# nianticlabs/wavelet-monodepth

Hardware: AMD Instinct MI355X
Metric: decoder+IDWT frames/sec @640x192 bs12 (higher is better)
Workload: dtype f32; 1 GPU; KITTI ResNet18 640x192 dense wavelet decoder + 4x Haar IDWT, forward, batch 12 per GPU (BASELINE.json configs[1]); encoder features resident in HBM; batch_per_gpu=12, global_batch=12, parallelism=dp1 (independent shards)

## Files before the change

### include/wmd.h

```cpp
#ifndef WMD_H
#define WMD_H

#include <stddef.h>
#include <stdint.h>

#ifdef __cplusplus
extern "C" {
#endif

#define WMD_VERSION 100

typedef enum {
    WMD_OK = 0,
    WMD_ERR_BAD_ARG = -1,
    WMD_ERR_BAD_SHAPE = -2,
    WMD_ERR_UNSUPPORTED = -3,
    WMD_ERR_HIP = -4,
    WMD_ERR_WORKSPACE = -5,
    WMD_ERR_COMM = -6
} wmd_status;

typedef enum { WMD_PAD_ZERO = 0, WMD_PAD_REFLECT = 1, WMD_PAD_REPLICATE = 2 } wmd_pad;

typedef enum { WMD_ACT_NONE = 0, WMD_ACT_ELU = 1, WMD_ACT_LEAKY = 2, WMD_ACT_SIGMOID = 3 } wmd_act;
// ... 27 lines not shown
    int B, H, W;
    int C1;
    int up1;
    int C2;
    int Cout;
    int ksize;
    int pad_mode;
    int act;
    float slope;
    const float* x1;
    const float* x2;
    const float* wp;
    const float* bias;
    float* y;
    float* workspace;
    size_t workspace_floats;
    int tune_cfg;
    int tune_ksplit;
    const float* wp_wino;
    const float* gate;
    int gate_act;
    float gate_slope;
    const uint8_t* in_mask;
    const uint8_t* out_mask;
    int in_mask_2x2;
    const int32_t* out_tiles;
    const int32_t* out_tile_count;
    int out_tile_h, out_tile_w;
} wmd_conv_args;

int wmd_conv_list_tile_supported(int tile_h, int tile_w);

int wmd_conv_fwd(const wmd_conv_args* args, void* stream);

size_t wmd_conv_fwd_workspace_floats(const wmd_conv_args* args);

size_t wmd_conv_packed_weight_floats_wino(int Cout, int Cin);
int wmd_conv_pack_weights_wino(const float* w, float* wp, int Cout, int Cin, int dgrad, void* stream);

typedef struct {
    const float* w;
    int Cout, Cin, ksize;
    float* fwd;
    float* dgrad;
    float* wino_fwd;
    float* wino_dgrad;
} wmd_pack_item;
int wmd_conv_pack_many(const wmd_pack_item* items, int n, void* stream);

int wmd_conv_num_configs(void);
const char* wmd_conv_config_name(int i);

size_t wmd_conv_bf16_packed_weight_bytes(int Cout, int Cin, int terms);
int wmd_conv_bf16_pack_weights(const float* w, void* wp, int Cout, int Cin, int terms, void* stream);
int wmd_conv_bf16_supported(const wmd_conv_args* args, int terms);
size_t wmd_conv_bf16_workspace_floats(const wmd_conv_args* args, int terms);
int wmd_conv_bf16_fwd(const wmd_conv_args* args, int terms, void* stream);
int wmd_conv_bf16_num_configs(void);
const char* wmd_conv_bf16_config_name(int i);

int wmd_act_bwd(const float* dy, const float* y, float* dz, size_t n, int act, float slope, void* stream);

typedef struct {
    int B, H, W;
    int C1, up1, C2, Cout, ksize, pad_mode;
    const float* dz;
    const float* wp_dgrad;
    float* dx1;
    float* dx2;
    float* workspace;
    size_t workspace_floats;
    int tune_cfg;
    int tune_ksplit;
    const float* wp_dgrad_wino;
    const float* x1_fwd;
    int x1_act;
    float x1_slope;
} wmd_conv_dgrad_args;

size_t wmd_conv_dgrad_workspace_floats(const wmd_conv_dgrad_args* args);
int wmd_conv_dgrad(const wmd_conv_dgrad_args* args, void* stream);

typedef struct {
    int B, H, W;
    int C1, up1, C2, Cout, ksize, pad_mode;
    const float* x1;
    const float* x2;
    const float* dz;
    float* dw;
    float* dbias;
    float* workspace;
    size_t workspace_floats;
    int tune_cfg;
    int tune_nsplit;
} wmd_conv_wgrad_args;

int wmd_conv_wgrad_num_configs(void);
const char* wmd_conv_wgrad_config_name(int index);

size_t wmd_conv_wgrad_workspace_floats(const wmd_conv_wgrad_args* args);
int wmd_conv_wgrad(const wmd_conv_wgrad_args* args, void* stream);

typedef struct {
    int B, H, W;
    int C1, up1, C2, pad_mode;
    const float* x1;
    const float* x2;
    const float* w;
} wmd_dwconv_args;
int wmd_dwconv3x3_fwd(const wmd_dwconv_args* args, float* y, void* stream);
size_t wmd_dwconv3x3_bwd_workspace_floats(const wmd_dwconv_args* args);
int wmd_dwconv3x3_bwd(const wmd_dwconv_args* args, const float* y, const float* dy, float* dx1, float* dx2, float* dw,
                      float* workspace, size_t workspace_floats, void* stream);

typedef struct {
    int B, H, W, C;
    int Cout;
    int pad_mode;
    int mode;
    float scale;
    const float* xp; const float* wgt_p; const float* bias_p;
    const float* xn; const float* wgt_n; const float* bias_n;
    float* y;
    float* sig_p;
    float* sig_n;
    size_t xp_bstride;
    size_t xn_bstride;
    float* workspace;
    size_t workspace_floats;
} wmd_head_args;

int wmd_head3x3_fwd(const wmd_head_args* args, void* stream);
size_t wmd_head3x3_workspace_floats(const wmd_head_args* args);

typedef struct {
    int B, H, W, C;
    float slope;
    const float* x;
    const float* wp1;
    const float* bias1;
    const float* wp2;
    float* t;
    int chain;
    int t_planes;
    const uint8_t* run_mask;
    const float* ll_wp1;
    const float* ll_bias1;
    const float* ll_wp2;
    float* mid_out;
    int mid_ct, mid_off_p, mid_off_n, mid_off_ll;
} wmd_head_fused_args;
int wmd_head_fused_fwd(const wmd_head_fused_args* args, void* stream);
int wmd_head_fused_multi_fwd(const wmd_head_fused_args* levels, int n_levels, void* stream);

typedef struct {
    int B, H, W;
    int pad_mode;
    float scale;
    const float* t;
    const float* bias_p;
    const float* bias_n;
    float* yh;
    const float* yl;
    float* out;
    float* disp;
    float disp_scale;
    int clamp01;
    const float* bias_ll;
    float scale_ll;
    float* yl_out;
    const uint8_t* yh_mask;
    uint32_t* range_keys;
    float* sig_p;
    float* sig_n;
    float* sig_ll;
} wmd_head_shiftsum_args;
int wmd_head_shiftsum_fwd(const wmd_head_shiftsum_args* args, void* stream);
int wmd_head_shiftsum_chain_fwd(const wmd_head_shiftsum_args* levels, int n_levels, void* stream);

typedef struct {
    int B, H, W, C;
    int pad_mode;
    float slope;
    float scale;
    const float* x;
    const float* wp1;
    const float* bias1;
    const float* wp2;
    const float* bias_p;
    const float* bias_n;
    float* yh;
    const float* yl;
    float* out;
    float* disp;
    float disp_scale;
    int clamp01;
    const uint8_t* yh_mask;
    float* mid_out;
    int mid_ct, mid_off_p, mid_off_n;
    float* sig_p;
    float* sig_n;
} wmd_head_level_args;
int wmd_head_level_supported(int C);
int wmd_head_level_fwd(const wmd_head_level_args* args, void* stream);
int wmd_head_level_pyramid_supported(int C, int B, int H, int W);
int wmd_head_level_pyramid_fwd(const wmd_head_level_args* args, const wmd_head_shiftsum_args* coarse, int n_coarse, void* stream);

typedef struct {
    int row0;
    int nrows;
    int ch0;
    int nch;
    const float* w3;
    float* dw3;
    float* db3;
} wmd_head_bwd_head;
typedef struct {
    int B, H, W;
    int Ct;
    int n_out;
    int pad_mode;
    int act;
    float slope;
    const float* dy3;
    const float* mid;
    float* dzmid;
    int n_heads;
    wmd_head_bwd_head head[3];
    float* workspace;
    size_t workspace_floats;
} wmd_head3x3_bwd_args;
size_t wmd_head3x3_bwd_workspace_floats(const wmd_head3x3_bwd_args* args);
int wmd_head3x3_bwd(const wmd_head3x3_bwd_args* args, void* stream);

typedef struct {
    int B, H, W;
    int C;
    int Ct;
    int x_act;
    float x_slope;
    const float* dz;
    const float* x;
    const float* w1;
    float* dx;
    float* dw1;
    float* db1;
    float* workspace;
    size_t workspace_floats;
} wmd_head1x1_bwd_args;
size_t wmd_head1x1_bwd_workspace_floats(const wmd_head1x1_bwd_args* args);
int wmd_head1x1_bwd(const wmd_head1x1_bwd_args* args, void* stream);
int wmd_head_bwd(const wmd_head3x3_bwd_args* a3, const wmd_head1x1_bwd_args* a1, void* stream);


int wmd_minmax(const float* x, size_t n, float* out2, void* stream);

int wmd_mask_threshold(const float* yh, const float* minmax, float thresh_ratio, uint8_t* mask,
                       int h, int w, void* stream);

typedef struct {
    int up;
    int radius;
    uint8_t* out;
    int32_t* nnz;
    int nnz_stride;
} wmd_dilate_spec;
int wmd_mask_dilate_multi(const uint8_t* mask, int h, int w, const wmd_dilate_spec* specs, int n, void* stream);
int wmd_mask_dilate_multi_b(const uint8_t* mask, int B, int h, int w, const wmd_dilate_spec* specs, int n, void* stream);

int wmd_mask_level(const float* yl, size_t n_yl, const float* yh, float thresh_ratio, int h, int w,
                   const wmd_dilate_spec* specs, int n, void* stream);
int wmd_mask_level_b(const float* yl, size_t n_yl, const float* yh, float thresh_ratio, int B, int h, int w,
                     const wmd_dilate_spec* specs, int n, float* minmax_scratch, void* stream);

typedef struct {
    int up, radius;
    uint8_t* out;
    int count;
    int tile_h, tile_w;
    int32_t* tile_list;
    int32_t* tile_count;
    const uint8_t* and_mask;
} wmd_level_spec;

typedef struct {
    int B, h, w;
    const float* yl;
    size_t n_yl;
    const float* yh;
    float thresh_ratio;
    const uint8_t* mask0;
    const float* minmax;
    uint32_t* range_keys;
    const wmd_level_spec* specs;
    int n;
    int32_t* scratch;
    int32_t* counts;
    int ring_slots, slot_ints, counts_off, ncounts;
    int advance;
} wmd_mask_level_args;
size_t wmd_mask_level_scratch_ints(int B);
int wmd_mask_level_lists(const wmd_mask_level_args* args, void* stream);

typedef struct {
    const uint8_t* mask;
    int npix;
// ... 99 lines not shown
```

### wavelet_monodepth_amd/_lib.py

```python
import ctypes as C
import os

_HERE = os.path.dirname(os.path.abspath(__file__))
LIB_PATH = os.environ.get("WMD_LIB_PATH") or os.path.join(_HERE, "libwmd_hip.so")

PAD = {"zero": 0, "constant": 0, "reflect": 1, "reflection": 1, "replicate": 2}
ACT = {"none": 0, None: 0, "elu": 1, "leaky": 2, "sigmoid": 3}


class WmdError(RuntimeError):
    pass


class ConvArgs(C.Structure):
    _fields_ = [("B", C.c_int), ("H", C.c_int), ("W", C.c_int), ("C1", C.c_int), ("up1", C.c_int), ("C2", C.c_int),
                ("Cout", C.c_int), ("ksize", C.c_int), ("pad_mode", C.c_int), ("act", C.c_int), ("slope", C.c_float),
                ("x1", C.c_void_p), ("x2", C.c_void_p), ("wp", C.c_void_p), ("bias", C.c_void_p), ("y", C.c_void_p),
                ("workspace", C.c_void_p), ("workspace_floats", C.c_size_t), ("tune_cfg", C.c_int), ("tune_ksplit", C.c_int),
                ("wp_wino", C.c_void_p), ("gate", C.c_void_p), ("gate_act", C.c_int), ("gate_slope", C.c_float),
                ("in_mask", C.c_void_p), ("out_mask", C.c_void_p), ("in_mask_2x2", C.c_int),
                ("out_tiles", C.c_void_p), ("out_tile_count", C.c_void_p), ("out_tile_h", C.c_int), ("out_tile_w", C.c_int)]


class ConvDgradArgs(C.Structure):
# ... 9 lines not shown
                ("Cout", C.c_int), ("ksize", C.c_int), ("pad_mode", C.c_int),
                ("x1", C.c_void_p), ("x2", C.c_void_p), ("dz", C.c_void_p), ("dw", C.c_void_p), ("dbias", C.c_void_p),
                ("workspace", C.c_void_p), ("workspace_floats", C.c_size_t), ("tune_cfg", C.c_int), ("tune_nsplit", C.c_int)]


class HeadArgs(C.Structure):
    _fields_ = [("B", C.c_int), ("H", C.c_int), ("W", C.c_int), ("C", C.c_int), ("Cout", C.c_int),
                ("pad_mode", C.c_int), ("mode", C.c_int), ("scale", C.c_float),
                ("xp", C.c_void_p), ("wgt_p", C.c_void_p), ("bias_p", C.c_void_p),
                ("xn", C.c_void_p), ("wgt_n", C.c_void_p), ("bias_n", C.c_void_p),
                ("y", C.c_void_p), ("sig_p", C.c_void_p), ("sig_n", C.c_void_p),
                ("xp_bstride", C.c_size_t), ("xn_bstride", C.c_size_t),
                ("workspace", C.c_void_p), ("workspace_floats", C.c_size_t)]


class HeadFusedArgs(C.Structure):
    _fields_ = [("B", C.c_int), ("H", C.c_int), ("W", C.c_int), ("C", C.c_int), ("slope", C.c_float),
                ("x", C.c_void_p), ("wp1", C.c_void_p), ("bias1", C.c_void_p), ("wp2", C.c_void_p), ("t", C.c_void_p),
                ("chain", C.c_int), ("t_planes", C.c_int), ("run_mask", C.c_void_p), ("ll_wp1", C.c_void_p),
                ("ll_bias1", C.c_void_p), ("ll_wp2", C.c_void_p), ("mid_out", C.c_void_p), ("mid_ct", C.c_int),
                ("mid_off_p", C.c_int), ("mid_off_n", C.c_int), ("mid_off_ll", C.c_int)]


class HeadLevelArgs(C.Structure):
    _fields_ = [("B", C.c_int), ("H", C.c_int), ("W", C.c_int), ("C", C.c_int), ("pad_mode", C.c_int),
                ("slope", C.c_float), ("scale", C.c_float),
                ("x", C.c_void_p), ("wp1", C.c_void_p), ("bias1", C.c_void_p), ("wp2", C.c_void_p),
                ("bias_p", C.c_void_p), ("bias_n", C.c_void_p), ("yh", C.c_void_p),
                ("yl", C.c_void_p), ("out", C.c_void_p), ("disp", C.c_void_p), ("disp_scale", C.c_float),
                ("clamp01", C.c_int), ("yh_mask", C.c_void_p), ("mid_out", C.c_void_p), ("mid_ct", C.c_int),
                ("mid_off_p", C.c_int), ("mid_off_n", C.c_int), ("sig_p", C.c_void_p), ("sig_n", C.c_void_p)]


class HeadBwdHead(C.Structure):
    _fields_ = [("row0", C.c_int), ("nrows", C.c_int), ("ch0", C.c_int), ("nch", C.c_int), ("w3", C.c_void_p),
                ("dw3", C.c_void_p), ("db3", C.c_void_p)]


class Head3x3BwdArgs(C.Structure):
    _fields_ = [("B", C.c_int), ("H", C.c_int), ("W", C.c_int), ("Ct", C.c_int), ("n_out", C.c_int), ("pad_mode", C.c_int),
                ("act", C.c_int), ("slope", C.c_float), ("dy3", C.c_void_p), ("mid", C.c_void_p), ("dzmid", C.c_void_p),
                ("n_heads", C.c_int), ("head", HeadBwdHead * 3), ("workspace", C.c_void_p), ("workspace_floats", C.c_size_t)]


class Head1x1BwdArgs(C.Structure):
    _fields_ = [("B", C.c_int), ("H", C.c_int), ("W", C.c_int), ("C", C.c_int), ("Ct", C.c_int), ("x_act", C.c_int),
                ("x_slope", C.c_float), ("dz", C.c_void_p), ("x", C.c_void_p), ("w1", C.c_void_p), ("dx", C.c_void_p),
                ("dw1", C.c_void_p), ("db1", C.c_void_p), ("workspace", C.c_void_p), ("workspace_floats", C.c_size_t)]


class EvalKittiArgs(C.Structure):
    _fields_ = [("B", C.c_int), ("h", C.c_int), ("w", C.c_int), ("H", C.c_int), ("W", C.c_int),
                ("min_depth", C.c_float), ("max_depth", C.c_float), ("mask_mode", C.c_int), ("pred_scale", C.c_float),
                ("median_scaling", C.c_int), ("pred_disp", C.c_void_p), ("gt_depth", C.c_void_p), ("out", C.c_void_p),
                ("workspace", C.c_void_p), ("workspace_floats", C.c_size_t)]


class WarpArgs(C.Structure):
    _fields_ = [("B", C.c_int), ("C", C.c_int), ("H", C.c_int), ("W", C.c_int), ("Hs", C.c_int), ("Ws", C.c_int),
                ("eps", C.c_float), ("src", C.c_void_p), ("depth", C.c_void_p), ("K", C.c_void_p), ("inv_K", C.c_void_p),
                ("T", C.c_void_p)]


class DwConvArgs(C.Structure):
    _fields_ = [("B", C.c_int), ("H", C.c_int), ("W", C.c_int), ("C1", C.c_int), ("up1", C.c_int), ("C2", C.c_int),
                ("pad_mode", C.c_int), ("x1", C.c_void_p), ("x2", C.c_void_p), ("w", C.c_void_p)]


class HeadShiftsumArgs(C.Structure):
    _fields_ = [("B", C.c_int), ("H", C.c_int), ("W", C.c_int), ("pad_mode", C.c_int), ("scale", C.c_float),
                ("t", C.c_void_p), ("bias_p", C.c_void_p), ("bias_n", C.c_void_p), ("yh", C.c_void_p),
                ("yl", C.c_void_p), ("out", C.c_void_p), ("disp", C.c_void_p), ("disp_scale", C.c_float),
                ("clamp01", C.c_int), ("bias_ll", C.c_void_p), ("scale_ll", C.c_float), ("yl_out", C.c_void_p),
                ("yh_mask", C.c_void_p), ("range_keys", C.c_void_p), ("sig_p", C.c_void_p), ("sig_n", C.c_void_p),
                ("sig_ll", C.c_void_p)]


class LevelSpec(C.Structure):
    _fields_ = [("up", C.c_int), ("radius", C.c_int), ("out", C.c_void_p), ("count", C.c_int), ("tile_h", C.c_int),
                ("tile_w", C.c_int), ("tile_list", C.c_void_p), ("tile_count", C.c_void_p), ("and_mask", C.c_void_p)]


class MaskLevelArgs(C.Structure):
    _fields_ = [("B", C.c_int), ("h", C.c_int), ("w", C.c_int), ("yl", C.c_void_p), ("n_yl", C.c_size_t), ("yh", C.c_void_p),
                ("thresh_ratio", C.c_float), ("mask0", C.c_void_p), ("minmax", C.c_void_p), ("range_keys", C.c_void_p),
                ("specs", C.POINTER(LevelSpec)), ("n", C.c_int), ("scratch", C.c_void_p), ("counts", C.c_void_p),
                ("ring_slots", C.c_int), ("slot_ints", C.c_int), ("counts_off", C.c_int), ("ncounts", C.c_int),
                ("advance", C.c_int)]


class DilateSpec(C.Structure):
    _fields_ = [("up", C.c_int), ("radius", C.c_int), ("out", C.c_void_p), ("nnz", C.c_void_p), ("nnz_stride", C.c_int)]


class PackItem(C.Structure):
    _fields_ = [("w", C.c_void_p), ("Cout", C.c_int), ("Cin", C.c_int), ("ksize", C.c_int), ("fwd", C.c_void_p),
                ("dgrad", C.c_void_p), ("wino_fwd", C.c_void_p), ("wino_dgrad", C.c_void_p)]


class CompactSpec(C.Structure):
    _fields_ = [("mask", C.c_void_p), ("npix", C.c_int), ("coords", C.c_void_p), ("nnz", C.c_void_p)]


class SparseConvArgs(C.Structure):
    _fields_ = [("H", C.c_int), ("W", C.c_int), ("C1", C.c_int), ("up1", C.c_int), ("C1tot", C.c_int), ("c1_off", C.c_int),
                ("C2", C.c_int), ("Cout", C.c_int), ("ksize", C.c_int), ("pad_mode", C.c_int), ("act", C.c_int),
                ("slope", C.c_float), ("x1", C.c_void_p), ("x2", C.c_void_p), ("in_mask", C.c_void_p),
                ("out_coords", C.c_void_p), ("out_nnz", C.c_void_p), ("max_out", C.c_int),
                ("wp", C.c_void_p), ("bias", C.c_void_p), ("wp2", C.c_void_p), ("bias2", C.c_void_p),
                ("c1_off2", C.c_int), ("out_scale", C.c_float), ("y", C.c_void_p), ("split_waves", C.c_int),
                ("B", C.c_int), ("nnz_stride", C.c_int)]


_lib = None

SIGNATURES = {
    "wmd_version": (C.c_int, []),
    "wmd_last_error": (C.c_char_p, []),
    "wmd_status_string": (C.c_char_p, [C.c_int]),
    "wmd_profile_begin": (C.c_int, []),
    "wmd_profile_end": (C.c_long, [C.c_char_p, C.c_size_t]),
    "wmd_idwt_haar_fwd": (C.c_int, [C.c_void_p] * 4 + [C.c_int] * 3 + [C.c_float, C.c_int, C.c_void_p]),
    "wmd_idwt_haar_bwd": (C.c_int, [C.c_void_p] * 5 + [C.c_int] * 3 + [C.c_float, C.c_int, C.c_void_p]),
    "wmd_dwt_haar_fwd": (C.c_int, [C.c_void_p] * 3 + [C.c_int] * 3 + [C.c_void_p]),
    "wmd_dwt_haar_reflect_fwd": (C.c_int, [C.c_void_p] * 3 + [C.c_int] * 3 + [C.c_void_p]),
    "wmd_conv_packed_weight_floats": (C.c_size_t, [C.c_int] * 3),
    "wmd_conv_pack_weights": (C.c_int, [C.c_void_p, C.c_void_p, C.c_int, C.c_int, C.c_int, C.c_void_p]),
    "wmd_conv_pack_weights_dgrad": (C.c_int, [C.c_void_p, C.c_void_p, C.c_int, C.c_int, C.c_int, C.c_void_p]),
    "wmd_conv_packed_weight_floats_wino": (C.c_size_t, [C.c_int, C.c_int]),
    "wmd_conv_pack_weights_wino": (C.c_int, [C.c_void_p, C.c_void_p, C.c_int, C.c_int, C.c_int, C.c_void_p]),
    "wmd_conv_pack_many": (C.c_int, [C.c_void_p, C.c_int, C.c_void_p]),
    "wmd_conv_fwd": (C.c_int, [C.POINTER(ConvArgs), C.c_void_p]),
    "wmd_conv_fwd_workspace_floats": (C.c_size_t, [C.POINTER(ConvArgs)]),
    "wmd_conv_num_configs": (C.c_int, []),
    "wmd_conv_config_name": (C.c_char_p, [C.c_int]),
    "wmd_conv_bf16_packed_weight_bytes": (C.c_size_t, [C.c_int] * 3),
    "wmd_conv_bf16_pack_weights": (C.c_int, [C.c_void_p, C.c_void_p, C.c_int, C.c_int, C.c_int, C.c_void_p]),
    "wmd_conv_bf16_supported": (C.c_int, [C.POINTER(ConvArgs), C.c_int]),
    "wmd_conv_bf16_workspace_floats": (C.c_size_t, [C.POINTER(ConvArgs), C.c_int]),
    "wmd_conv_bf16_fwd": (C.c_int, [C.POINTER(ConvArgs), C.c_int, C.c_void_p]),
    "wmd_conv_bf16_num_configs": (C.c_int, []),
    "wmd_conv_bf16_config_name": (C.c_char_p, [C.c_int]),
    "wmd_act_bwd": (C.c_int, [C.c_void_p] * 3 + [C.c_size_t, C.c_int, C.c_float, C.c_void_p]),
    "wmd_conv_dgrad_workspace_floats": (C.c_size_t, [C.POINTER(ConvDgradArgs)]),
    "wmd_conv_dgrad": (C.c_int, [C.POINTER(ConvDgradArgs), C.c_void_p]),
    "wmd_conv_wgrad_workspace_floats": (C.c_size_t, [C.POINTER(ConvWgradArgs)]),
    "wmd_conv_wgrad": (C.c_int, [C.POINTER(ConvWgradArgs), C.c_void_p]),
    "wmd_conv_wgrad_num_configs": (C.c_int, []),
    "wmd_conv_wgrad_config_name": (C.c_char_p, [C.c_int]),
    "wmd_head3x3_fwd": (C.c_int, [C.POINTER(HeadArgs), C.c_void_p]),
    "wmd_head3x3_workspace_floats": (C.c_size_t, [C.POINTER(HeadArgs)]),
    "wmd_head_fused_fwd": (C.c_int, [C.POINTER(HeadFusedArgs), C.c_void_p]),
    "wmd_head_fused_multi_fwd": (C.c_int, [C.POINTER(HeadFusedArgs), C.c_int, C.c_void_p]),
    "wmd_head_shiftsum_fwd": (C.c_int, [C.POINTER(HeadShiftsumArgs), C.c_void_p]),
    "wmd_head_shiftsum_chain_fwd": (C.c_int, [C.POINTER(HeadShiftsumArgs), C.c_int, C.c_void_p]),
    "wmd_head_level_supported": (C.c_int, [C.c_int]),
    "wmd_head_level_fwd": (C.c_int, [C.POINTER(HeadLevelArgs), C.c_void_p]),
    "wmd_head_level_pyramid_supported": (C.c_int, [C.c_int, C.c_int, C.c_int, C.c_int]),
    "wmd_head_level_pyramid_fwd": (C.c_int, [C.POINTER(HeadLevelArgs), C.POINTER(HeadShiftsumArgs), C.c_int, C.c_void_p]),
    "wmd_head3x3_bwd_workspace_floats": (C.c_size_t, [C.POINTER(Head3x3BwdArgs)]),
    "wmd_head3x3_bwd": (C.c_int, [C.POINTER(Head3x3BwdArgs), C.c_void_p]),
    "wmd_head1x1_bwd_workspace_floats": (C.c_size_t, [C.POINTER(Head1x1BwdArgs)]),
    "wmd_head1x1_bwd": (C.c_int, [C.POINTER(Head1x1BwdArgs), C.c_void_p]),
    "wmd_head_bwd": (C.c_int, [C.POINTER(Head3x3BwdArgs), C.POINTER(Head1x1BwdArgs), C.c_void_p]),
    "wmd_minmax": (C.c_int, [C.c_void_p, C.c_size_t, C.c_void_p, C.c_void_p]),
    "wmd_mask_threshold": (C.c_int, [C.c_void_p, C.c_void_p, C.c_float, C.c_void_p, C.c_int, C.c_int, C.c_void_p]),
    "wmd_mask_dilate_multi": (C.c_int, [C.c_void_p, C.c_int, C.c_int, C.POINTER(DilateSpec), C.c_int, C.c_void_p]),
    "wmd_mask_level": (C.c_int, [C.c_void_p, C.c_size_t, C.c_void_p, C.c_float, C.c_int, C.c_int, C.POINTER(DilateSpec), C.c_int,
                       C.c_void_p]),
    "wmd_mask_compact_multi": (C.c_int, [C.POINTER(CompactSpec), C.c_int, C.c_void_p]),
    "wmd_mask_dilate_multi_b": (C.c_int, [C.c_void_p, C.c_int, C.c_int, C.c_int, C.POINTER(DilateSpec), C.c_int, C.c_void_p]),
    "wmd_mask_level_b": (C.c_int, [C.c_void_p, C.c_size_t, C.c_void_p, C.c_float, C.c_int, C.c_int, C.c_int, C.POINTER(DilateSpec), C.c_int,
                         C.c_void_p, C.c_void_p]),
    "wmd_mask_compact_multi_b": (C.c_int, [C.POINTER(CompactSpec), C.c_int, C.c_int, C.c_void_p]),
    "wmd_mask_level_scratch_ints": (C.c_size_t, [C.c_int]),
    "wmd_mask_level_lists": (C.c_int, [C.POINTER(MaskLevelArgs), C.c_void_p]),
    "wmd_conv_list_tile_supported": (C.c_int, [C.c_int, C.c_int]),
    "wmd_sparse_conv": (C.c_int, [C.POINTER(SparseConvArgs), C.c_void_p]),
    "wmd_upsample_bilinear_fwd": (C.c_int, [C.c_void_p] * 3 + [C.c_int] * 6 + [C.c_float, C.c_float, C.c_void_p]),
    "wmd_upsample_bilinear_bwd": (C.c_int, [C.c_void_p] * 4 + [C.c_int] * 6 + [C.c_float, C.c_float, C.c_void_p]),
    "wmd_eval_workspace_floats": (C.c_size_t, [C.c_int, C.c_int, C.c_int]),
    "wmd_eval_kitti": (C.c_int, [C.POINTER(EvalKittiArgs), C.c_void_p]),
    "wmd_eval_errors": (C.c_int, [C.c_void_p, C.c_void_p, C.c_int, C.c_size_t, C.c_void_p, C.c_void_p]),
    "wmd_flip_postprocess": (C.c_int, [C.c_void_p, C.c_void_p, C.c_void_p, C.c_int, C.c_int, C.c_int, C.c_void_p]),
    "wmd_ssim_fwd": (C.c_int, [C.c_void_p] * 3 + [C.c_int] * 5 + [C.c_float, C.c_float, C.c_void_p]),
    "wmd_ssim_bwd_workspace_floats": (C.c_size_t, [C.c_int] * 4),
    "wmd_ssim_bwd": (C.c_int, [C.c_void_p] * 5 + [C.c_int] * 5 + [C.c_float, C.c_float, C.c_void_p, C.c_size_t, C.c_void_p]),
    "wmd_warp_fwd": (C.c_int, [C.POINTER(WarpArgs), C.c_void_p, C.c_void_p]),
    "wmd_warp_bwd_workspace_floats": (C.c_size_t, [C.POINTER(WarpArgs)]),
    "wmd_warp_bwd": (C.c_int, [C.POINTER(WarpArgs), C.c_void_p, C.c_void_p, C.c_void_p, C.c_void_p, C.c_size_t, C.c_void_p]),
    "wmd_smooth_workspace_floats": (C.c_size_t, [C.c_int] * 3),
    "wmd_smooth_fwd": (C.c_int, [C.c_void_p] * 3 + [C.c_int] * 4 + [C.c_float, C.c_void_p, C.c_size_t, C.c_void_p]),
    "wmd_smooth_bwd": (C.c_int, [C.c_void_p] * 4 + [C.c_int] * 4 + [C.c_float, C.c_void_p]),
    "wmd_dwconv3x3_fwd": (C.c_int, [C.POINTER(DwConvArgs), C.c_void_p, C.c_void_p]),
    "wmd_dwconv3x3_bwd_workspace_floats": (C.c_size_t, [C.POINTER(DwConvArgs)]),
    "wmd_dwconv3x3_bwd": (C.c_int, [C.POINTER(DwConvArgs)] + [C.c_void_p] * 6 + [C.c_size_t, C.c_void_p]),
    "wmd_comm_unique_id": (C.c_int, [C.c_void_p]),
    "wmd_comm_init": (C.c_int, [C.POINTER(C.c_void_p), C.c_void_p, C.c_int, C.c_int]),
    "wmd_comm_allreduce": (C.c_int, [C.c_void_p, C.c_void_p, C.c_size_t, C.c_float, C.c_void_p]),
    "wmd_comm_broadcast": (C.c_int, [C.c_void_p, C.c_void_p, C.c_size_t, C.c_int, C.c_void_p]),
    "wmd_comm_info": (C.c_int, [C.c_void_p, C.POINTER(C.c_int), C.POINTER(C.c_int), C.POINTER(C.c_int)]),
    "wmd_comm_destroy": (C.c_int, [C.c_void_p]),
}


def lib():
    global _lib
    if _lib is None:
        if not os.path.exists(LIB_PATH):
            raise WmdError("%s not found: build it with `python -m wavelet_monodepth_amd.build` "
                           "(or __graft_entry__.build()); there is no CPU fallback" % LIB_PATH)
        handle = C.CDLL(LIB_PATH)
        for name, (res, args) in SIGNATURES.items():
            fn = getattr(handle, name)
            fn.restype = res
            fn.argtypes = args
        _lib = handle
    return _lib


def check(status, what=""):
    if status != 0:
        l = lib()
        raise WmdError("%s failed: %s (%s)" % (what or "libwmd_hip call", l.wmd_status_string(status).decode(),
                                               l.wmd_last_error().decode()))


def ptr(t):
    if t is None:
        return None
    if not t.is_cuda:
        raise WmdError("libwmd_hip expects device tensors, got a %s tensor" % t.device)
    assert t.is_contiguous(), "libwmd_hip expects contiguous tensors"
    return t.data_ptr()


def current_stream():
    import torch

    return torch.cuda.current_stream().cuda_stream


def profile_begin():
    check(lib().wmd_profile_begin(), "wmd_profile_begin")


def profile_end():
    import json

    buf = C.create_string_buffer(1 << 16)
    n = lib().wmd_profile_end(buf, len(buf))
    if n < 0:
        check(int(n), "wmd_profile_end")
    return json.loads(buf.value.decode())
```

### wavelet_monodepth_amd/csrc/wmd_head_chain.hip

```cpp
#include <algorithm>
#include <cstdlib>
#include <type_traits>
#include <utility>
#include "wmd_internal.h"

#ifndef WMD_CHAIN_PD256
#define WMD_CHAIN_PD256 4
#endif
#ifndef WMD_CHAIN_PD128
#define WMD_CHAIN_PD128 1
#endif

namespace wmd {

typedef float f32x4 __attribute__((ext_vector_type(4)));

template <class F, int... I>
__device__ __forceinline__ void hc_static_for_impl(F&& f, std::integer_sequence<int, I...>) {
    (f(std::integral_constant<int, I>{}), ...);
}
template <int N, class F>
__device__ __forceinline__ void hc_static_for(F&& f) {
    hc_static_for_impl(f, std::make_integer_sequence<int, N>{});
}

__device__ __forceinline__ void hc_barrier() {
    asm volatile("s_waitcnt lgkmcnt(0)" ::: "memory");
    __builtin_amdgcn_s_barrier();
    asm volatile("" ::: "memory");
}

struct HeadChainArgs {
    const float* x;
    const float* wp1;
    const float* bias1;
    const float* wp2;
    float* t;
    int plane, tiles, t_planes;
    int C;
    float slope;
    const uint8_t* run_mask;
    const float* ll_wp1;
    const float* ll_bias1;
    const float* ll_wp2;
    float* mid_out;
    int mid_ct, mid_off[3];
};

template <int C, int RS, int PG, int NT, int KC>
struct HeadChainTile {
    static constexpr int NW = RS * PG, NTH = NW * 64;
    static constexpr int PXB = PG * NT * 16;
    static constexpr int MTS = C / 16;
    static constexpr int MT = MTS / RS;
    static constexpr int KS = C / 4;
    static constexpr int NCH = KS / KC;
    static constexpr int XS = PXB % 32 == 0 ? PXB + 16 : PXB + 32;
    static constexpr int WF = MTS * KC * 64;
    static constexpr int XF = KC * 4 * XS;
    static constexpr int NBUF = NCH > 1 ? 2 : 1;
    static constexpr int WV = (WF / 4 + NTH - 1) / NTH;
    static constexpr int XV = (KC * PXB + NTH - 1) / NTH;
    static constexpr int RED = RS > 1 ? NW * 3 * NT * 256 : 0;
    static constexpr int WFL = (C == 256 && RS == 4) ? RS * KC * 64 : 0;
    static constexpr int STAGE = NBUF * (WF + WFL + XF);
    static constexpr int LDS_FLOATS = STAGE > RED ? STAGE : RED;
    static_assert(C % 16 == 0 && MTS % RS == 0 && KS % KC == 0, "whole tiles");
    static_assert(XS % 32 == 16 && PXB % 4 == 0, "bank-conflict-free x rows");
};

template <class T, int KC, bool LLX>
__device__ __forceinline__ void chain_fetch(f32x4 (&wreg)[T::WV], f32x4 (&xreg)[T::XV], f32x4& lreg, const float* __restrict__ w1,
                                            const float* __restrict__ wl, const float* __restrict__ xb, int c, int tid, int pix0, int plane) {
    if constexpr (LLX) {
        static_assert(T::WFL > 0 && T::WFL / 4 <= T::NTH, "one 16-byte piece per thread covers the low-pass part of a chunk");
        const int f = tid * 4, m = f / (KC * 64), rem = f % (KC * 64);
        if (f < T::WFL) lreg = *reinterpret_cast<const f32x4*>(wl + ((size_t)m * T::KS + c * KC) * 64 + rem);
    }
#pragma unroll
    for (int v = 0; v < T::WV; ++v) {
        const int f = (v * T::NTH + tid) * 4;
        const int m = f / (KC * 64), rem = f % (KC * 64);
        f32x4 wv = {0.f, 0.f, 0.f, 0.f};
        if (T::WF % (4 * T::NTH) == 0 || f < T::WF) wv = *reinterpret_cast<const f32x4*>(w1 + ((size_t)m * T::KS + c * KC) * 64 + rem);
        wreg[v] = wv;
    }
#pragma unroll
    for (int v = 0; v < T::XV; ++v) {
        const int q = v * T::NTH + tid;
        const int chl = q / (T::PXB / 4), px = pix0 + (q % (T::PXB / 4)) * 4;
        f32x4 val = {0.f, 0.f, 0.f, 0.f};
        if (q < KC * T::PXB && px < plane)
            val = *reinterpret_cast<const f32x4*>(xb + (size_t)(c * KC * 4 + chl) * plane + px);
        xreg[v] = val;
    }
}

template <class T, int KC, bool LLX>
__device__ __forceinline__ void chain_commit(const f32x4 (&wreg)[T::WV], const f32x4 (&xreg)[T::XV], const f32x4& lreg, float* ws, int tid) {
    float* xs = ws + T::WF + T::WFL;
    if constexpr (LLX) {
        if (tid * 4 < T::WFL) *reinterpret_cast<f32x4*>(ws + T::WF + tid * 4) = lreg;
    }
#pragma unroll
    for (int v = 0; v < T::WV; ++v)
        if (T::WF % (4 * T::NTH) == 0 || (v * T::NTH + tid) * 4 < T::WF) *reinterpret_cast<f32x4*>(ws + (v * T::NTH + tid) * 4) = wreg[v];
#pragma unroll
    for (int v = 0; v < T::XV; ++v) {
        const int q = v * T::NTH + tid;
        if (q < KC * T::PXB) *reinterpret_cast<f32x4*>(xs + (q / (T::PXB / 4)) * T::XS + (q % (T::PXB / 4)) * 4) = xreg[v];
    }
}

template <int C, int RS, int PG, int NT, int KC, bool LLX, int PD>
__device__ __forceinline__ void head_chain_body(const HeadChainArgs& a, float* lds, const int bx, const int side) {
    using T = HeadChainTile<C, RS, PG, NT, KC>;
    constexpr int MT = T::MT, KS = T::KS, XS = T::XS, PXB = T::PXB;
    constexpr int MTX = MT + (LLX ? 1 : 0);
    static_assert(!LLX || (C / 4) / 16 == RS, "the low-pass chain: C/4 mid channels = one row tile per channel slice");

    const int tid = threadIdx.x, lane = tid & 63;
    const int wave = __builtin_amdgcn_readfirstlane(tid >> 6);
    const int r = wave % RS, pg = wave / RS;
    const int g = lane >> 4, lc = lane & 15;
    const int tile = bx % a.tiles, b = bx / a.tiles;
    const int pix0 = tile * PXB, plane = a.plane;
    if (a.run_mask) {
        static_assert(PXB <= T::NTH, "one mask byte per thread covers the block's pixel run");
        __shared__ int run_any[T::NW];
        const bool mine = tid < PXB && pix0 + tid < plane && a.run_mask[(size_t)b * plane + pix0 + tid] != 0;
        const bool wave_any = __builtin_amdgcn_ballot_w64(mine) != 0;
        if (lane == 0) run_any[wave] = wave_any ? 1 : 0;
        __syncthreads();
        int all = 0;
#pragma unroll
        for (int w = 0; w < T::NW; ++w) all |= run_any[w];
        if (all == 0) return;
    }
    const float* xb = a.x + (size_t)b * C * plane;
    const float* w1 = a.wp1 + (size_t)side * T::MTS * KS * 64;
    const float* w2 = a.wp2 + (size_t)side * 2 * KS * 64;

    static_assert(PD >= 1 && (T::NCH % PD == 0 || T::NCH == 1), "the chunk loop is unrolled by the prefetch distance");
    f32x4 wreg[PD][T::WV], xreg[PD][T::XV], lreg[PD];
#pragma unroll
    for (int d = 0; d < PD; ++d) lreg[d] = f32x4{0.f, 0.f, 0.f, 0.f};
    constexpr int BUF = T::WF + T::WFL + T::XF;

    f32x4 acc[MTX][NT];
#pragma unroll
    for (int m = 0; m < MTX; ++m)
#pragma unroll
        for (int n = 0; n < NT; ++n) acc[m][n] = f32x4{0.f, 0.f, 0.f, 0.f};

    chain_fetch<T, KC, LLX>(wreg[0], xreg[0], lreg[0], w1, a.ll_wp1, xb, 0, tid, pix0, plane);
    chain_commit<T, KC, LLX>(wreg[0], xreg[0], lreg[0], lds, tid);
    hc_static_for<PD>([&](auto kc) __attribute__((always_inline)) {
        constexpr int k = decltype(kc)::value + 1;
        if (k < T::NCH) chain_fetch<T, KC, LLX>(wreg[k % PD], xreg[k % PD], lreg[k % PD], w1, a.ll_wp1, xb, k, tid, pix0, plane);
    });
    hc_barrier();
    for (int c0 = 0; c0 < T::NCH; c0 += PD) {
        hc_static_for<PD>([&](auto dc) __attribute__((always_inline)) {
            constexpr int d = decltype(dc)::value, dn = (d + 1) % PD;
            const int c = c0 + d;
            const float* ws = lds + (c & (T::NBUF - 1)) * BUF;
            const float* xs = ws + T::WF + T::WFL;
#pragma unroll
            for (int kk = 0; kk < KC; ++kk) {
                float xf[NT], wf[MTX];
#pragma unroll
                for (int n = 0; n < NT; ++n) xf[n] = xs[(kk * 4 + g) * XS + (pg * NT + n) * 16 + lc];
#pragma unroll
                for (int m = 0; m < MT; ++m) wf[m] = ws[((r * MT + m) * KC + kk) * 64 + lane];
                if constexpr (LLX) wf[MT] = ws[T::WF + (r * KC + kk) * 64 + lane];
#pragma unroll
                for (int m = 0; m < MTX; ++m)
#pragma unroll
                    for (int n = 0; n < NT; ++n) acc[m][n] = __builtin_amdgcn_mfma_f32_16x16x4f32(wf[m], xf[n], acc[m][n], 0, 0, 0);
            }
            if (c + 1 < T::NCH) {
                chain_commit<T, KC, LLX>(wreg[dn], xreg[dn], lreg[dn], lds + ((c + 1) & (T::NBUF - 1)) * BUF, tid);
                if (c + 1 + PD < T::NCH)
                    chain_fetch<T, KC, LLX>(wreg[dn], xreg[dn], lreg[dn], w1, a.ll_wp1, xb, c + 1 + PD, tid, pix0, plane);
                hc_barrier();
            }
        });
    }

    f32x4 acc2[2][NT];
#pragma unroll
    for (int j = 0; j < 2; ++j)
#pragma unroll
        for (int n = 0; n < NT; ++n) acc2[j][n] = f32x4{0.f, 0.f, 0.f, 0.f};
#pragma unroll
    for (int m = 0; m < MT; ++m) {
        const int mg = r * MT + m;
        float bv[4] = {0.f, 0.f, 0.f, 0.f};
        if (a.bias1) {
            const float4 b4 = *reinterpret_cast<const float4*>(a.bias1 + side * C + mg * 16 + g * 4);
            bv[0] = b4.x, bv[1] = b4.y, bv[2] = b4.z, bv[3] = b4.w;
        }
        float w2f[2][4];
#pragma unroll
        for (int j = 0; j < 2; ++j)
#pragma unroll
            for (int i = 0; i < 4; ++i) w2f[j][i] = w2[((size_t)j * KS + 4 * mg + g) * 64 + i * 16 + lc];
#pragma unroll
        for (int i = 0; i < 4; ++i) {
#pragma unroll
            for (int n = 0; n < NT; ++n) {
                const float mid = act_apply(acc[m][n][i] + bv[i], WMD_ACT_LEAKY, a.slope);
                if (a.mid_out) {
                    const int px = pix0 + (pg * NT + n) * 16 + lc;
                    if (px < plane) a.mid_out[((size_t)b * a.mid_ct + a.mid_off[side] + mg * 16 + g * 4 + i) * plane + px] = mid;
                }
#pragma unroll
                for (int j = 0; j < 2; ++j) acc2[j][n] = __builtin_amdgcn_mfma_f32_16x16x4f32(w2f[j][i], mid, acc2[j][n], 0, 0, 0);
            }
        }
    }

    f32x4 acc2l[NT];
#pragma unroll
    for (int n = 0; n < NT; ++n) acc2l[n] = f32x4{0.f, 0.f, 0.f, 0.f};
    if constexpr (LLX) {
        float bv[4] = {0.f, 0.f, 0.f, 0.f};
        if (a.ll_bias1) {
            const float4 b4 = *reinterpret_cast<const float4*>(a.ll_bias1 + r * 16 + g * 4);
            bv[0] = b4.x, bv[1] = b4.y, bv[2] = b4.z, bv[3] = b4.w;
        }
        float w2l[4];
#pragma unroll
        for (int i = 0; i < 4; ++i) w2l[i] = a.ll_wp2[((size_t)4 * r + g) * 64 + i * 16 + lc];
#pragma unroll
        for (int i = 0; i < 4; ++i)
#pragma unroll
            for (int n = 0; n < NT; ++n) {
                const float mid = act_apply(acc[MT][n][i] + bv[i], WMD_ACT_LEAKY, a.slope);
                if (a.mid_out) {
                    const int px = pix0 + (pg * NT + n) * 16 + lc;
                    if (px < plane) a.mid_out[((size_t)b * a.mid_ct + a.mid_off[2] + r * 16 + g * 4 + i) * plane + px] = mid;
                }
                acc2l[n] = __builtin_amdgcn_mfma_f32_16x16x4f32(w2l[i], mid, acc2l[n], 0, 0, 0);
            }
    }

    if constexpr (RS > 1) {
        constexpr int NJ = LLX ? 3 : 2;
        __syncthreads();
        float* red = lds + (size_t)wave * 3 * NT * 256;
#pragma unroll
        for (int j = 0; j < NJ; ++j)
#pragma unroll
            for (int n = 0; n < NT; ++n) {
                const f32x4 v = j < 2 ? acc2[j < 2 ? j : 0][n] : acc2l[n];
                *reinterpret_cast<float4*>(red + ((j * NT + n) * 64 + lane) * 4) = make_float4(v[0], v[1], v[2], v[3]);
            }
        __syncthreads();
        if (r != 0) return;
#pragma unroll
        for (int j = 0; j < NJ; ++j)
#pragma unroll
            for (int n = 0; n < NT; ++n) {
                float4 s = *reinterpret_cast<const float4*>(lds + (size_t)(pg * RS) * 3 * NT * 256 + ((j * NT + n) * 64 + lane) * 4);
#pragma unroll
                for (int rr = 1; rr < RS; ++rr) {
                    const float4 p = *reinterpret_cast<const float4*>(lds + (size_t)(pg * RS + rr) * 3 * NT * 256 + ((j * NT + n) * 64 + lane) * 4);
                    s.x += p.x, s.y += p.y, s.z += p.z, s.w += p.w;
                }
                if (j < 2) acc2[j < 2 ? j : 0][n] = f32x4{s.x, s.y, s.z, s.w};
                else acc2l[n] = f32x4{s.x, s.y, s.z, s.w};
            }
    }

    float* tb = a.t + ((size_t)b * a.t_planes + side * 27) * plane;
#pragma unroll
    for (int n = 0; n < NT; ++n) {
        const int px = pix0 + (pg * NT + n) * 16 + lc;
        if (px >= plane) continue;
#pragma unroll
        for (int j = 0; j < 2; ++j)
#pragma unroll
            for (int i = 0; i < 4; ++i) {
                const int row = j * 16 + g * 4 + i;
                if (row < 27) tb[(size_t)row * plane + px] = acc2[j][n][i];
            }
        if constexpr (LLX) {
#pragma unroll
            for (int i = 0; i < 4; ++i) {
                const int row = g * 4 + i;
                if (row < 9) tb[(size_t)(54 + row) * plane + px] = acc2l[n][i];
            }
        }
    }
}

template <int C, int RS, int PG, int NT, int KC, int PD, bool LLC = false>
__global__ __launch_bounds__(RS* PG * 64, (RS * PG >= 8 ? 3 : 1)) void head_chain_kernel(const HeadChainArgs a) {
    using T = HeadChainTile<C, RS, PG, NT, KC>;
    __shared__ __attribute__((aligned(16))) float lds[T::LDS_FLOATS];
    if constexpr (LLC) {
        if (blockIdx.y == 0) {
            head_chain_body<C, RS, PG, NT, KC, true, PD>(a, lds, blockIdx.x, 0);
            return;
        }
    }
    head_chain_body<C, RS, PG, NT, KC, false, PD>(a, lds, blockIdx.x, blockIdx.y);
}

struct HeadChainMulti {
    HeadChainArgs lv[3];
    int first[4];
    int n;
};
constexpr int head_chain_multi_lds() {
    int m = HeadChainTile<256, 4, 1, 1, 4>::LDS_FLOATS;
    if (HeadChainTile<128, 1, 4, 1, 8>::LDS_FLOATS > m) m = HeadChainTile<128, 1, 4, 1, 8>::LDS_FLOATS;
    if (HeadChainTile<64, 1, 4, 2, 16>::LDS_FLOATS > m) m = HeadChainTile<64, 1, 4, 2, 16>::LDS_FLOATS;
    return m;
}
__global__ __launch_bounds__(256, 3) void head_chain_multi_kernel(const HeadChainMulti m) {
    __shared__ __attribute__((aligned(16))) float lds[head_chain_multi_lds()];
    int k = 0;
    while (k + 1 < m.n && (int)blockIdx.x >= m.first[k + 1]) ++k;
    const HeadChainArgs& a = m.lv[k];
    const int v = (int)blockIdx.x - m.first[k], per_side = (m.first[k + 1] - m.first[k]) >> 1;
    const int side = v >= per_side ? 1 : 0, bx = v - side * per_side;
    if (a.C == 256) {
        if (side == 0 && a.ll_wp1) head_chain_body<256, 4, 1, 1, 4, true, WMD_CHAIN_PD256>(a, lds, bx, 0);
        else head_chain_body<256, 4, 1, 1, 4, false, WMD_CHAIN_PD256>(a, lds, bx, side);
    } else if (a.C == 128) {
        head_chain_body<128, 1, 4, 1, 8, false, WMD_CHAIN_PD128>(a, lds, bx, side);
    } else {
        head_chain_body<64, 1, 4, 2, 16, false, 1>(a, lds, bx, side);
    }
}

template <int C, int RS, int PG, int NT, int KC, int PD>
static void launch_chain(const HeadChainArgs& a, int B, hipStream_t s) {
    using T = HeadChainTile<C, RS, PG, NT, KC>;
    HeadChainArgs k = a;
    k.tiles = (a.plane + T::PXB - 1) / T::PXB;
    if constexpr (C == 256 && RS == 4) {
        if (a.ll_wp1) {
            hipLaunchKernelGGL((head_chain_kernel<C, RS, PG, NT, KC, PD, true>), dim3((unsigned)(B * k.tiles), 2), dim3(T::NTH), 0, s, k);
            return;
        }
    }
    hipLaunchKernelGGL((head_chain_kernel<C, RS, PG, NT, KC, PD>), dim3((unsigned)(B * k.tiles), 2), dim3(T::NTH), 0, s, k);
}

static HeadChainArgs head_chain_args(const wmd_head_fused_args* g, int t_planes, long plane, bool& with_ll) {
    HeadChainArgs a;
    a.x = g->x;
    a.wp1 = g->wp1;
    a.bias1 = g->bias1;
    a.wp2 = g->wp2;
    a.t = g->t;
    a.plane = (int)plane;
    a.tiles = 0;
    a.t_planes = t_planes;
    a.slope = g->slope;
    a.run_mask = g->run_mask;
    with_ll = g->ll_wp1 && g->ll_wp2 && g->C == 256 && t_planes == 81 && !g->run_mask;
    a.ll_wp1 = with_ll ? g->ll_wp1 : nullptr;
    a.ll_bias1 = with_ll ? g->ll_bias1 : nullptr;
    a.ll_wp2 = with_ll ? g->ll_wp2 : nullptr;
    a.mid_out = g->mid_out;
    a.mid_ct = g->mid_ct;
    a.mid_off[0] = g->mid_off_p;
    a.mid_off[1] = g->mid_off_n;
    a.mid_off[2] = g->mid_off_ll;
    a.C = g->C;
    return a;
}

int head_chain_launch(const wmd_head_fused_args* g, int t_planes, hipStream_t s) {
    static const bool on = [] {
        const char* e = getenv("WMD_HEAD_CHAIN");
        return !(e && atoi(e) == 0);
    }();
    const long plane = (long)g->H * g->W;
    if (!on || (plane & 3) || plane > (1L << 28) || (g->C != 64 && g->C != 128 && g->C != 256)) return 0;
    bool with_ll = false;
    HeadChainArgs a = head_chain_args(g, t_planes, plane, with_ll);
    const double pix = (double)g->B * plane;
    ProfScope prof("head_chain_kernel", 2.0 * pix * (2.0 * g->C * g->C + 54.0 * g->C), 4.0 * pix * (g->C + 54), s);
    if (g->C == 64)
        launch_chain<64, 1, 4, 2, 16, 1>(a, g->B, s);
    else if (g->C == 128)
        launch_chain<128, 1, 4, 1, 8, WMD_CHAIN_PD128>(a, g->B, s);
    else {
        static const int pg_force = [] {
            const char* e = getenv("WMD_HEAD_CHAIN_PG256");
            return e ? atoi(e) : 0;
        }();
        const long b32 = (long)g->B * ((plane + 31) / 32) * 2, b48 = (long)g->B * ((plane + 47) / 48) * 2;
        const long cost32 = ((b32 + kNumCU - 1) / kNumCU) * 2, cost48 = ((b48 + kNumCU - 1) / kNumCU) * 3;
        if (pg_force == 3 || (pg_force == 0 && cost48 < cost32)) launch_chain<256, 4, 3, 1, 4, WMD_CHAIN_PD256>(a, g->B, s);
        else launch_chain<256, 4, 2, 1, 4, WMD_CHAIN_PD256>(a, g->B, s);
    }
    return with_ll ? 2 : 1;
}

int head_chain_multi_launch(const wmd_head_fused_args* g, int n, hipStream_t s) {
    static const bool on = [] {
        const char* e = getenv("WMD_HEAD_CHAIN_MULTI");
        const char* c = getenv("WMD_HEAD_CHAIN");
        return !(e && atoi(e) == 0) && !(c && atoi(c) == 0);
    }();
    if (!on || n < 1 || n > 3) return 0;
    HeadChainMulti m;
    m.n = n;
    m.first[0] = 0;
    double flops = 0, bytes = 0;
    for (int k = 0; k < n; ++k) {
        const long plane = (long)g[k].H * g[k].W;
        const int t_planes = g[k].t_planes ? g[k].t_planes : 54;
        if ((plane & 3) || plane > (1L << 28) || (g[k].C != 64 && g[k].C != 128 && g[k].C != 256) || g[k].run_mask || g[k].mid_out || g[k].chain != 0)
            return 0;
        if (g[k].ll_wp1 && (g[k].C != 256 || t_planes != 81 || !g[k].ll_wp2)) return 0;
        bool with_ll = false;
        m.lv[k] = head_chain_args(&g[k], t_planes, plane, with_ll);
        const int pxb = g[k].C == 256 ? 16 : (g[k].C == 128 ? 64 : 128);
        m.lv[k].tiles = (int)((plane + pxb - 1) / pxb);
        const long blocks = 2L * g[k].B * m.lv[k].tiles;
        if (m.first[k] + blocks > (1L << 30)) return 0;
        m.first[k + 1] = m.first[k] + (int)blocks;
        const double pix = (double)g[k].B * plane;
        flops += 2.0 * pix * (2.0 * g[k].C * g[k].C + 54.0 * g[k].C);
        bytes += 4.0 * pix * (g[k].C + 54);
    }
    ProfScope prof("head_chain_multi_kernel", flops, bytes, s);
    hipLaunchKernelGGL(head_chain_multi_kernel, dim3((unsigned)m.first[n]), dim3(256), 0, s, m);
    return n;
}

}
```

Measured before the change: 23890 frames/s.

## Add persistent register-resident-weight path for C=64 head chain level

Adds a persistent-block variant of the C=64 head chain inside the multi-level kernel. Each wave keeps its conv weights in registers, loops over 16-pixel groups with a grid stride, and double-buffers the next group's input loads behind the MFMA work using buffer loads. The persistent level is placed first in the block ordering by default, so the large early level overlaps with other levels' blocks. The aim is to cut repeated weight loads and launch-tile overhead for the largest-resolution level, at the cost of heavy register use and fewer blocks in flight, which can starve load balancing.

Measured after the change: 23800 frames/s. About the same (-0.4%).

```diff
diff --git a/include/wmd.h b/include/wmd.h
--- a/include/wmd.h
+++ b/include/wmd.h
@@ -203,6 +203,7 @@
 } wmd_head_fused_args;
 int wmd_head_fused_fwd(const wmd_head_fused_args* args, void* stream);
 int wmd_head_fused_multi_fwd(const wmd_head_fused_args* levels, int n_levels, void* stream);
+int wmd_head_chain_persist_blocks(void);
 
 typedef struct {
     int B, H, W;
diff --git a/wavelet_monodepth_amd/_lib.py b/wavelet_monodepth_amd/_lib.py
--- a/wavelet_monodepth_amd/_lib.py
+++ b/wavelet_monodepth_amd/_lib.py
@@ -185,6 +185,7 @@
     "wmd_head3x3_workspace_floats": (C.c_size_t, [C.POINTER(HeadArgs)]),
     "wmd_head_fused_fwd": (C.c_int, [C.POINTER(HeadFusedArgs), C.c_void_p]),
     "wmd_head_fused_multi_fwd": (C.c_int, [C.POINTER(HeadFusedArgs), C.c_int, C.c_void_p]),
+    "wmd_head_chain_persist_blocks": (C.c_int, []),
     "wmd_head_shiftsum_fwd": (C.c_int, [C.POINTER(HeadShiftsumArgs), C.c_void_p]),
     "wmd_head_shiftsum_chain_fwd": (C.c_int, [C.POINTER(HeadShiftsumArgs), C.c_int, C.c_void_p]),
     "wmd_head_level_supported": (C.c_int, [C.c_int]),
diff --git a/wavelet_monodepth_amd/csrc/wmd_head_chain.hip b/wavelet_monodepth_amd/csrc/wmd_head_chain.hip
--- a/wavelet_monodepth_amd/csrc/wmd_head_chain.hip
+++ b/wavelet_monodepth_amd/csrc/wmd_head_chain.hip
@@ -9,6 +9,9 @@
 #endif
 #ifndef WMD_CHAIN_PD128
 #define WMD_CHAIN_PD128 1
+#endif
+#ifndef WMD_CHAIN_PERSIST_PER_CU
+#define WMD_CHAIN_PERSIST_PER_CU 1
 #endif
 
 namespace wmd {
@@ -296,6 +299,116 @@
     }
 }
 
+__device__ __forceinline__ __amdgpu_buffer_rsrc_t hc_x_rsrc(const HeadChainArgs& a, int b) {
+    return __builtin_amdgcn_make_buffer_rsrc(const_cast<float*>(a.x + (size_t)b * 64 * a.plane), 0, 64 * a.plane * 4, 0x00020000);
+}
+__device__ __forceinline__ float hc_x_load(__amdgpu_buffer_rsrc_t r, int lane_off, int row_off) {
+    return __builtin_bit_cast(float, __builtin_amdgcn_raw_buffer_load_b32(r, lane_off, row_off, 0));
+}
+
+template <bool MORE>
+__device__ __forceinline__ void head_chain_persist_step(float (&xr)[16], const float (&w1f)[4][16], const float (&w2f)[2][4][4], const float* bias_lds,
+                                                        const HeadChainArgs& a, const int side, const int grp, const int nxt, const int g, const int lc) {
+    constexpr int KS = 16, MT = 4;
+    const int plane = a.plane;
+    __amdgpu_buffer_rsrc_t rn = hc_x_rsrc(a, 0);
+    int offn = 0;
+    if constexpr (MORE) {
+        const int bn = nxt / a.tiles, tn = nxt - bn * a.tiles;
+        rn = hc_x_rsrc(a, bn);
+        offn = (g * plane + min(tn * 16 + lc, plane - 1)) * 4;
+    }
+    f32x4 acc[MT];
+#pragma unroll
+    for (int m = 0; m < MT; ++m) acc[m] = f32x4{0.f, 0.f, 0.f, 0.f};
+#pragma unroll
+    for (int kk = 0; kk < KS; ++kk) {
+#pragma unroll
+        for (int m = 0; m < MT; ++m) acc[m] = __builtin_amdgcn_mfma_f32_16x16x4f32(w1f[m][kk], xr[kk], acc[m], 0, 0, 0);
+        if constexpr (MORE) xr[kk] = hc_x_load(rn, offn, kk * 16 * plane);
+    }
+    f32x4 acc2[2];
+    acc2[0] = acc2[1] = f32x4{0.f, 0.f, 0.f, 0.f};
+#pragma unroll
+    for (int m = 0; m < MT; ++m) {
+        const float4 b4 = *reinterpret_cast<const float4*>(bias_lds + m * 16 + g * 4);
+        const float bv[4] = {b4.x, b4.y, b4.z, b4.w};
+#pragma unroll
+        for (int i = 0; i < 4; ++i) {
+            const float mid = act_apply(acc[m][i] + bv[i], WMD_ACT_LEAKY, a.slope);
+#pragma unroll
+            for (int j = 0; j < 2; ++j) acc2[j] = __builtin_amdgcn_mfma_f32_16x16x4f32(w2f[j][m][i], mid, acc2[j], 0, 0, 0);
+        }
+    }
+    const int b = grp / a.tiles, tile = grp - b * a.tiles, px = tile * 16 + lc;
+    const __amdgpu_buffer_rsrc_t rt =
+        __builtin_amdgcn_make_buffer_rsrc(a.t + ((size_t)b * a.t_planes + side * 27) * plane, 0, 27 * plane * 4, 0x00020000);
+    const int offt = (g * 4 * plane + px) * 4;
+    if (px < plane) {
+#pragma unroll
+        for (int j = 0; j < 2; ++j)
+#pragma unroll
+            for (int i = 0; i < 4; ++i)
+                if (j * 16 + g * 4 + i < 27) {
+                    const float v = acc2[j][i];
+                    __builtin_amdgcn_raw_buffer_store_b32(__builtin_bit_cast(unsigned, v), rt, offt, (j * 16 + i) * plane * 4, 0);
+                }
+    }
+}
+
+__device__ __forceinline__ void head_chain_persist_body(const HeadChainArgs& a, float* lds, const int blk, const int nblk, const int groups) {
+    constexpr int C = 64, KS = 16, MT = 4;
+    const int lane = threadIdx.x & 63, g = lane >> 4, lc = lane & 15;
+    const int wave = __builtin_amdgcn_readfirstlane(threadIdx.x >> 6);
+    const int side = wave & 1, Q = 2 * nblk;
+    int grp = 2 * blk + (wave >> 1);
+    if (grp >= groups) return;
+    const int plane = a.plane;
+
+    float xr[2][KS];
+    hc_static_for<2>([&](auto dc) __attribute__((always_inline)) {
+        constexpr int d = decltype(dc)::value;
+        const int gr = d == 0 ? grp : min(grp + Q, groups - 1);
+        const int b = gr / a.tiles, tile = gr - b * a.tiles;
+        const __amdgpu_buffer_rsrc_t r = hc_x_rsrc(a, b);
+        const int off = (g * plane + min(tile * 16 + lc, plane - 1)) * 4;
+#pragma unroll
+        for (int kk = 0; kk < KS; ++kk) xr[d][kk] = hc_x_load(r, off, kk * 16 * plane);
+    });
+
+    const float* w1 = a.wp1 + (size_t)side * MT * KS * 64;
+    const float* w2 = a.wp2 + (size_t)side * 2 * KS * 64;
+    float w1f[MT][KS], w2f[2][MT][4];
+#pragma unroll
+    for (int m = 0; m < MT; ++m) {
+#pragma unroll
+        for (int kk = 0; kk < KS; ++kk) w1f[m][kk] = w1[(m * KS + kk) * 64 + lane];
+#pragma unroll
+        for (int j = 0; j < 2; ++j)
+#pragma unroll
+            for (int i = 0; i < 4; ++i) w2f[j][m][i] = w2[((size_t)j * KS + 4 * m + g) * 64 + i * 16 + lc];
+    }
+    float* bias_lds = lds + wave * C;
+    bias_lds[lane] = a.bias1 ? a.bias1[side * C + lane] : 0.f;
+    __builtin_amdgcn_fence(__ATOMIC_RELEASE, "wavefront");
+    __builtin_amdgcn_wave_barrier();
+    __builtin_amdgcn_fence(__ATOMIC_ACQUIRE, "wavefront");
+
+    for (;;) {
+        bool done = false;
+        hc_static_for<2>([&](auto dc) __attribute__((always_inline)) {
+            constexpr int d = decltype(dc)::value;
+            if (done) return;
+            const int nxt = grp + 2 * Q;
+            if (nxt < groups) head_chain_persist_step<true>(xr[d], w1f, w2f, bias_lds, a, side, grp, nxt, g, lc);
+            else head_chain_persist_step<false>(xr[d], w1f, w2f, bias_lds, a, side, grp, nxt, g, lc);
+            grp += Q;
+            if (grp >= groups) done = true;
+        });
+        if (done) break;
+    }
+}
+
 template <int C, int RS, int PG, int NT, int KC, int PD, bool LLC = false>
 __global__ __launch_bounds__(RS* PG * 64, (RS * PG >= 8 ? 3 : 1)) void head_chain_kernel(const HeadChainArgs a) {
     using T = HeadChainTile<C, RS, PG, NT, KC>;
@@ -313,6 +426,7 @@
     HeadChainArgs lv[3];
     int first[4];
     int n;
+    int pgroups;
 };
 constexpr int head_chain_multi_lds() {
     int m = HeadChainTile<256, 4, 1, 1, 4>::LDS_FLOATS;
@@ -332,6 +446,8 @@
         else head_chain_body<256, 4, 1, 1, 4, false, WMD_CHAIN_PD256>(a, lds, bx, side);
     } else if (a.C == 128) {
         head_chain_body<128, 1, 4, 1, 8, false, WMD_CHAIN_PD128>(a, lds, bx, side);
+    } else if (m.pgroups > 0) {
+        head_chain_persist_body(a, lds, v, m.first[k + 1] - m.first[k], m.pgroups);
     } else {
         head_chain_body<64, 1, 4, 2, 16, false, 1>(a, lds, bx, side);
     }
@@ -404,30 +520,71 @@
     return with_ll ? 2 : 1;
 }
 
+static int head_chain_persist_blocks() {
+    static const int blocks = [] {
+        const char* e = getenv("WMD_HEAD_CHAIN_PERSIST");
+        int per_cu = e ? atoi(e) : WMD_CHAIN_PERSIST_PER_CU;
+        if (per_cu <= 0) return 0;
+        int dev = 0, cus = 0, resident = 0;
+        if (hipGetDevice(&dev) != hipSuccess || hipDeviceGetAttribute(&cus, hipDeviceAttributeMultiprocessorCount, dev) != hipSuccess ||
+            hipOccupancyMaxActiveBlocksPerMultiprocessor(&resident, head_chain_multi_kernel, 256, 0) != hipSuccess || cus <= 0 || resident <= 0) {
+            (void)hipGetLastError();
+            return 0;
+        }
+        return cus * std::min(per_cu, resident);
+    }();
+    return blocks;
+}
+
 int head_chain_multi_launch(const wmd_head_fused_args* g, int n, hipStream_t s) {
     static const bool on = [] {
         const char* e = getenv("WMD_HEAD_CHAIN_MULTI");
         const char* c = getenv("WMD_HEAD_CHAIN");
         return !(e && atoi(e) == 0) && !(c && atoi(c) == 0);
     }();
+    static const bool persist_last = [] {
+        const char* e = getenv("WMD_HEAD_CHAIN_PERSIST_LAST");
+        return e && atoi(e) != 0;
+    }();
     if (!on || n < 1 || n > 3) return 0;
-    HeadChainMulti m;
-    m.n = n;
-    m.first[0] = 0;
-    double flops = 0, bytes = 0;
     for (int k = 0; k < n; ++k) {
         const long plane = (long)g[k].H * g[k].W;
         const int t_planes = g[k].t_planes ? g[k].t_planes : 54;
         if ((plane & 3) || plane > (1L << 28) || (g[k].C != 64 && g[k].C != 128 && g[k].C != 256) || g[k].run_mask || g[k].mid_out || g[k].chain != 0)
             return 0;
         if (g[k].ll_wp1 && (g[k].C != 256 || t_planes != 81 || !g[k].ll_wp2)) return 0;
+    }
+    const int pblocks = head_chain_persist_blocks();
+    int pk = -1;
+    for (int k = 0; k < n && pk < 0; ++k)
+        if (pblocks > 0 && g[k].C == 64 && (long)g[k].H * g[k].W <= (1L << 22) && (long)g[k].B * (((long)g[k].H * g[k].W + 15) / 16) < (1L << 30)) pk = k;
+    int order[3], no = 0;
+    if (pk >= 0 && !persist_last) order[no++] = pk;
+    for (int k = 0; k < n; ++k)
+        if (k != pk) order[no++] = k;
+    if (pk >= 0 && persist_last) order[no++] = pk;
+    HeadChainMulti m;
+    m.n = n;
+    m.first[0] = 0;
+    m.pgroups = 0;
+    double flops = 0, bytes = 0;
+    for (int o = 0; o < n; ++o) {
+        const int k = order[o];
+        const long plane = (long)g[k].H * g[k].W;
         bool with_ll = false;
-        m.lv[k] = head_chain_args(&g[k], t_planes, plane, with_ll);
-        const int pxb = g[k].C == 256 ? 16 : (g[k].C == 128 ? 64 : 128);
-        m.lv[k].tiles = (int)((plane + pxb - 1) / pxb);
-        const long blocks = 2L * g[k].B * m.lv[k].tiles;
-        if (m.first[k] + blocks > (1L << 30)) return 0;
-        m.first[k + 1] = m.first[k] + (int)blocks;
+        m.lv[o] = head_chain_args(&g[k], g[k].t_planes ? g[k].t_planes : 54, plane, with_ll);
+        long blocks;
+        if (k == pk) {
+            m.lv[o].tiles = (int)((plane + 15) / 16);
+            m.pgroups = g[k].B * m.lv[o].tiles;
+            blocks = pblocks;
+        } else {
+            const int pxb = g[k].C == 256 ? 16 : (g[k].C == 128 ? 64 : 128);
+            m.lv[o].tiles = (int)((plane + pxb - 1) / pxb);
+            blocks = 2L * g[k].B * m.lv[o].tiles;
+        }
+        if (m.first[o] + blocks > (1L << 30)) return 0;
+        m.first[o + 1] = m.first[o] + (int)blocks;
         const double pix = (double)g[k].B * plane;
         flops += 2.0 * pix * (2.0 * g[k].C * g[k].C + 54.0 * g[k].C);
         bytes += 4.0 * pix * (g[k].C + 54);
@@ -438,3 +595,5 @@
 }
 
 }
+
+extern "C" int wmd_head_chain_persist_blocks(void) { return wmd::head_chain_persist_blocks(); }
```
